# rafaelhuntstokes/bayesian_optimisation

Measured on AMD Instinct MI355X. Metric: candidate acquisitions/sec, higher is better.
Workload: dtype f64

## Files before the change

bayesian_optimisation_amd/_lib.py:

```python
from __future__ import annotations

import ctypes as C
import os

_HERE = os.path.dirname(os.path.abspath(__file__))
LIB_PATH = os.environ.get("GPBO_LIB") or os.path.join(_HERE, "libgpbo.so")

GPBO_OK = 0
ACQ_LCB = 0
ACQ_EI = 1
NPAD = 128
CHUNK_GRANULE = 512
MAX_D = 16
MAX_D_ANY = 1024
I8_MAX_N = 16384
BATCH_MAX_Q = 64
FANTASY_BELIEVER = 0
FANTASY_LIE = 1
REFINE_MAX_P = 4096
TS_MAX_PATHS = 64
TS_MAX_FEATURES = 16384
HYPER_MEAN = 1
HYPER_SCALE = 2
HYPER_CELLS_MAX_N = 64
# ... 48 lines not shown
    "gpbo_qei_workspace_bytes": (_i64, [_i64, _i64, _i64]),
    "gpbo_posterior_qei_f64": (C.c_int, [_p, _i64, _p, _i64, _i64, _i32, _p, _p, _p, _f64, _f64, _f64, _p, _i32, _i64,
                                         _i64, _p, _p, _p, _i64, _p, _p]),
    "gpbo_padded_n_f32": (_i64, [_i64]),
    "gpbo_prepare_f32": (C.c_int, [_p, _p, _i64, _p, _p, _i64, _p]),
    "gpbo_posterior_workspace_bytes_f32": (_i64, [_i64, _i64, _i64]),
    "gpbo_posterior_acq_f32": (C.c_int, [_p, _i64, _p, _i64, _i64, _i32, _p, _p, _p, _f64, _i32, _f64, _f64, _f64,
                                         _i64, _i64, _p, _p, _p, _p, _p, _p, _i64, _p, _p]),
    "gpbo_prepare_i8_bytes": (_i64, [_i64]),
    "gpbo_prepare_i8": (C.c_int, [_p, _i64, _p, _i64, _p]),
    "gpbo_posterior_workspace_bytes_i8": (_i64, [_i64, _i64, _i64]),
    "gpbo_posterior_acq_i8": (C.c_int, [_p, _i64, _p, _i64, _i64, _i32, _p, _p, _p, _f64, _i32, _f64, _f64, _i64, _i64,
                                        _p, _p, _p, _p, _p, _p, _i64, _p, _p]),
    "gpbo_posterior_acq_i8c": (C.c_int, [_p, _i64, _p, _i64, _i64, _i32, _p, _p, _p, _f64, _i32, _f64, _f64, _i64, _i64,
                                         _p, _p, _p, _p, _p, _p, _i64, _p, _p]),
    "gpbo_posterior_prefix_f64": (C.c_int, [_p, _i64, _p, _i64, _i64, _i32, _p, _p, _p, _f64, _i32, _f64, _f64, _i64, _i64,
                                            _i64, _p, _p, _p, _p, _p, _i64, _p, _p]),
    "gpbo_bound_select_f64": (C.c_int, [_p, _i64, _p, _p, _i64, _i64, _i32, _p, _p, _p, _f64, _i32, _f64, _f64, _i64,
                                        _i64, _i64, _i64, _i64, _p, _p, _p, _i64, _p]),
    "gpbo_fps_order_workspace_bytes": (_i64, [_i64]),
    "gpbo_fps_order_f64": (C.c_int, [_p, _p, _i64, _i32, _p, _i64, _p, _p, _p, _p, _i64, _p]),
    "gpbo_fps_order_status": (C.c_int, [_p, _i64, _p, _p]),
    "gpbo_rescore_workspace_bytes": (_i64, [_i64, _i64, _i64]),
    "gpbo_rescore_f64": (C.c_int, [_p, _i64, _p, _p, _p, _i64, _i64, _i32, _p, _p, _p, _f64, _i32, _f64, _f64, _i64,
                                   _f64, _i64, _i64, _i64, _p, _p, _p, _i64, _p]),
    "gpbo_batch_workspace_bytes": (_i64, [_i64, _i64, _i32]),
    "gpbo_select_batch_f64": (C.c_int, [_p, _i64, _p, _i64, _i64, _i32, _p, _p, _p, _f64, _f64, _f64, _i32, _f64, _f64, _i32,
                                        _i32, _f64, _p, _p, _i64, _p, _p, _p, _p, _p, _i64, _p]),
    "gpbo_select_batch_host_f64": (C.c_int, [_p, _p, _i64, _i32, _p, _f64, _f64, _p, _i64, _i32, _f64, _f64, _i64, _i32, _i32,
                                             _f64, _p, _p, _p, _p, _p, _p]),
    "gpbo_posterior_grad_workspace_bytes": (_i64, [_i64, _i64]),
    "gpbo_posterior_grad_f64": (C.c_int, [_p, _i64, _p, _i64, _i64, _i32, _p, _p, _p, _f64, _i32, _f64, _f64, _p, _p, _p, _p, _p,
                                          _p, _p, _i64, _p]),
    "gpbo_refine_workspace_bytes": (_i64, [_i64, _i64]),
    "gpbo_refine_f64": (C.c_int, [_p, _i64, _p, _p, _p, _i64, _i64, _i32, _p, _p, _p, _f64, _i32, _f64, _f64, _i32, _f64, _p, _p,
                                  _p, _p, _p, _p, _i64, _p]),
    "gpbo_refine_host_f64": (C.c_int, [_p, _p, _i64, _i32, _p, _f64, _f64, _p, _i64, _p, _p, _i32, _f64, _f64, _i32, _f64, _p, _p,
                                       _p, _p, _p, _p]),
    "gpbo_thompson_weights_workspace_bytes": (_i64, [_i64, _i32, _i32]),
    "gpbo_thompson_weights_f64": (C.c_int, [_p, _p, _i64, _i64, _i32, _p, _p, _f64, _f64, _p, _p, _p, _p, _i32, _i32, _p, _p, _i64,
                                            _p]),
    "gpbo_thompson_paths_workspace_bytes": (_i64, [_i64, _i64, _i32, _i32]),
    "gpbo_thompson_paths_f64": (C.c_int, [_p, _i64, _p, _i64, _i64, _i32, _p, _p, _p, _p, _p, _i32, _i32, _i64, _p, _i64, _p, _p,
                                          _p, _p, _i64, _p]),
    "gpbo_thompson_host_f64": (C.c_int, [_p, _p, _i64, _i32, _p, _f64, _f64, _p, _i64, _p, _p, _p, _p, _i32, _i32, _p, _p, _p, _p,
                                         _p]),
# ... 119 lines not shown
```

bayesian_optimisation_amd/csrc/rescore.hip:

```cpp
#include "gpbo_internal.h"

#include <limits>

namespace {

constexpr int SB = 256;

__device__ __forceinline__ void bounds(int kind, double mu, double var, double tau, double p0, double p1, double &lo,
                                       double &hi) {
    const double a = fabs(var);
    const double s_lo = sqrt(fmax(a - tau, 0.0)), s_hi = sqrt(a + tau);
    const double a_lo = gpbo_acquisition(kind, mu, s_lo, p0, p1);
    const double a_hi = gpbo_acquisition(kind, mu, s_hi, p0, p1);
    lo = (a_hi < a_lo) ? a_hi : a_lo;
    hi = (a_hi < a_lo) ? a_lo : a_hi;
}

__global__ __launch_bounds__(SB) void screen_lo_kernel(const double *__restrict__ mu, const double *__restrict__ var,
                                                       int64_t M, double tau, int kind, double p0, double p1,
                                                       double *__restrict__ part) {
    __shared__ double s_val[SB / 64];
    double best = -std::numeric_limits<double>::infinity();
    for (int64_t c = (int64_t)blockIdx.x * SB + threadIdx.x; c < M; c += (int64_t)gridDim.x * SB) {
        double lo, hi;
// ... 35 lines not shown
    const int lane = threadIdx.x & 63;
    const int64_t step = (int64_t)gridDim.x * SB;
    const int64_t cmax = (M + step - 1) / step * step;
    for (int64_t c = (int64_t)blockIdx.x * SB + threadIdx.x; c < cmax; c += step) {
        bool keep = false;
        if (c < M) {
            double lo, hi;
            bounds(kind, mu[c], var[c], tau, p0, p1, lo, hi);
            keep = !(hi < thr) || (c % stride) == 0;
        }
        const unsigned long long m = __ballot(keep);
        if (m) {
            unsigned long long base = 0;
            if (lane == 0) base = atomicAdd(count, (unsigned long long)__popcll(m));
            base = __shfl(base, 0);
            if (keep) {
                const unsigned long long pos = base + __popcll(m & ((1ull << lane) - 1ull));
                if ((int64_t)pos < cap) list[pos] = c;
            }
        }
    }
}

__global__ __launch_bounds__(SB) void bound_select_kernel(const double *__restrict__ ub, int64_t M, double thr, double slack,
                                                          int64_t stride, int64_t *__restrict__ list, int64_t cap,
                                                          unsigned long long *__restrict__ count) {
    __shared__ unsigned s_cnt[SB];
    __shared__ unsigned long long s_base;
    const int64_t step = (int64_t)gridDim.x * SB;
    unsigned mine = 0;
    for (int64_t c = (int64_t)blockIdx.x * SB + threadIdx.x; c < M; c += step)
        mine += (!(ub[c] + slack < thr) || (c % stride) == 0) ? 1u : 0u;
    s_cnt[threadIdx.x] = mine;
    __syncthreads();
    if (threadIdx.x == 0) {
        unsigned tot = 0;
        for (int t = 0; t < SB; ++t) { const unsigned v = s_cnt[t]; s_cnt[t] = tot; tot += v; }
        s_base = tot ? atomicAdd(count, (unsigned long long)tot) : 0ull;
    }
    __syncthreads();
    if (!list || !mine) return;
    unsigned long long pos = s_base + s_cnt[threadIdx.x];
    for (int64_t c = (int64_t)blockIdx.x * SB + threadIdx.x; c < M; c += step)
        if (!(ub[c] + slack < thr) || (c % stride) == 0) {
            if ((int64_t)pos < cap) list[pos] = c;
            ++pos;
        }
}

__global__ __launch_bounds__(SB) void bound_minmax_kernel(const double *__restrict__ ub, int64_t M, double *__restrict__ part) {
    __shared__ double s_hi[SB / 64], s_lo[SB / 64];
    double hi = -std::numeric_limits<double>::infinity(), lo = std::numeric_limits<double>::infinity();
    for (int64_t c = (int64_t)blockIdx.x * SB + threadIdx.x; c < M; c += (int64_t)gridDim.x * SB) {
        const double v = ub[c];
        if (v > hi) hi = v;
        if (v < lo) lo = v;
    }
#pragma unroll
    for (int off = 1; off < 64; off <<= 1) {
        hi = fmax(hi, __shfl_xor(hi, off));
        lo = fmin(lo, __shfl_xor(lo, off));
    }
    if ((threadIdx.x & 63) == 0) { s_hi[threadIdx.x >> 6] = hi; s_lo[threadIdx.x >> 6] = lo; }
    __syncthreads();
    if (threadIdx.x == 0) {
        for (int w = 1; w < SB / 64; ++w) { hi = fmax(hi, s_hi[w]); lo = fmin(lo, s_lo[w]); }
        part[blockIdx.x] = hi;
        part[gridDim.x + blockIdx.x] = lo;
    }
}

__global__ __launch_bounds__(SB) void bound_minmax_finish_kernel(const double *__restrict__ part, int n, double *__restrict__ out2) {
    __shared__ double s_hi[SB / 64], s_lo[SB / 64];
    double hi = -std::numeric_limits<double>::infinity(), lo = std::numeric_limits<double>::infinity();
    for (int i = threadIdx.x; i < n; i += SB) { hi = fmax(hi, part[i]); lo = fmin(lo, part[n + i]); }
#pragma unroll
    for (int off = 1; off < 64; off <<= 1) {
        hi = fmax(hi, __shfl_xor(hi, off));
        lo = fmin(lo, __shfl_xor(lo, off));
    }
    if ((threadIdx.x & 63) == 0) { s_hi[threadIdx.x >> 6] = hi; s_lo[threadIdx.x >> 6] = lo; }
    __syncthreads();
    if (threadIdx.x == 0) {
        for (int w = 1; w < SB / 64; ++w) { hi = fmax(hi, s_hi[w]); lo = fmin(lo, s_lo[w]); }
        out2[0] = hi;
        out2[1] = lo;
    }
}

__global__ __launch_bounds__(SB) void bound_refine_kernel(const double *__restrict__ ub2, const int64_t *__restrict__ list,
                                                          int64_t K, double thr, double slack, int64_t *__restrict__ list_out,
                                                          unsigned long long *__restrict__ count) {
    const int lane = threadIdx.x & 63;
    const int64_t step = (int64_t)gridDim.x * SB;
    const int64_t imax = (K + step - 1) / step * step;
    for (int64_t i = (int64_t)blockIdx.x * SB + threadIdx.x; i < imax; i += step) {
        const bool keep = i < K && !(ub2[i] + slack < thr);
        const unsigned long long m = __ballot(keep);
        if (m) {
            unsigned long long base = 0;
            if (lane == 0) base = atomicAdd(count, (unsigned long long)__popcll(m));
            base = __shfl(base, 0);
            if (keep) list_out[base + __popcll(m & ((1ull << lane) - 1ull))] = list[i];
        }
    }
}

__global__ __launch_bounds__(SB) void gather_rows_kernel(const double *__restrict__ Xs, int d, const int64_t *__restrict__ list,
                                                         int64_t K, double *__restrict__ out) {
    const int64_t e = (int64_t)blockIdx.x * SB + threadIdx.x;
    if (e >= K * d) return;
    const int64_t i = e / d;
    out[e] = Xs[list[i] * d + (e - i * d)];
}

// ... 28 lines not shown
        err = fmax(err, __shfl_xor(err, off));
        nans += __shfl_xor(nans, off);
    }
    const int w = threadIdx.x >> 6;
    if ((threadIdx.x & 63) == 0) { s_err[w] = err; s_nan[w] = nans; }
    gpbo_argmax_post(bv, bi, threadIdx.x & 63, w, s_val, s_idx);
    __syncthreads();
    if (threadIdx.x == 0) {
        gpbo_argmax_fold(s_val, s_idx, SB / 64, bv, bi);
        for (int q = 1; q < SB / 64; ++q) {
            err = fmax(err, s_err[q]);
            nans += s_nan[q];
        }
        out->res.best_val = bv;
        out->res.best_idx = bi;
        out->res.nan_count = (int64_t)nans;
        out->res.reserved = 0;
        out->err_max = err;
        out->pad = 0.0;
    }
}

struct RescoreLayout {
    int64_t part_off, L_off, count_off, list_off, rows_off, mu_off, sig_off, acq_off, out_off, post_off, post_bytes, total;
};

constexpr int SCREEN_BLOCKS = 1024;

RescoreLayout rescore_layout(int64_t Np, int64_t cap, int64_t chunk64) {
    RescoreLayout L;
    int64_t off = 0;
    L.part_off = off; off += align_up((int64_t)sizeof(double) * SCREEN_BLOCKS, 256);
    L.L_off = off; off += 256;
    L.count_off = off; off += 256;
    L.out_off = off; off += 256;
    L.list_off = off; off += align_up((int64_t)sizeof(int64_t) * cap, 256);
    L.rows_off = off; off += align_up((int64_t)sizeof(double) * cap * GPBO_MAX_D, 256);
    L.mu_off = off; off += align_up((int64_t)sizeof(double) * cap, 256);
    L.sig_off = off; off += align_up((int64_t)sizeof(double) * cap, 256);
    L.acq_off = off; off += align_up((int64_t)sizeof(double) * cap, 256);
    L.post_off = off;
    L.post_bytes = gpbo_posterior_workspace_bytes_split(Np, chunk64, cap, GPBO_RESCORE_SPLIT_MAX);
    off += align_up(L.post_bytes, 256);
    L.total = off;
    return L;
}

struct RescoreWork {
    double *part, *Ldev;
    unsigned long long *count;
    RescoreOut *out;
    int64_t *list;
    double *rows, *mu64, *sig64, *acq64;
    void *post;
    int64_t post_bytes;
    RescoreWork(void *work, const RescoreLayout &L) {
        char *w = reinterpret_cast<char *>(work);
        part = reinterpret_cast<double *>(w + L.part_off);
        Ldev = reinterpret_cast<double *>(w + L.L_off);
        count = reinterpret_cast<unsigned long long *>(w + L.count_off);
        out = reinterpret_cast<RescoreOut *>(w + L.out_off);
        list = reinterpret_cast<int64_t *>(w + L.list_off);
        rows = reinterpret_cast<double *>(w + L.rows_off);
        mu64 = reinterpret_cast<double *>(w + L.mu_off);
        sig64 = reinterpret_cast<double *>(w + L.sig_off);
        acq64 = reinterpret_cast<double *>(w + L.acq_off);
        post = w + L.post_off;
        post_bytes = L.post_bytes;
    }
};

bool read_back(void *dst_host, const void *src, size_t bytes, hipStream_t st) {
    return hipMemcpyAsync(dst_host, src, bytes, hipMemcpyDeviceToHost, st) == hipSuccess &&
           hipStreamSynchronize(st) == hipSuccess;
}

int score_list(const double *Xs, const GpModel &gp, const Acquisition &acq, int64_t chunk64, const RescoreWork &W, int64_t K,
               int64_t n_prefix, const DenseOut &dense, void *stream) {
    const int64_t tot = K * gp.d;
    hipLaunchKernelGGL(gather_rows_kernel, dim3((unsigned)((tot + SB - 1) / SB)), dim3(SB), 0, gpbo_stream(stream), Xs,
                       (int)gp.d, W.list, K, W.rows);
    GPBO_CHECK_LAUNCH();
    return gpbo_posterior_acq_f64_split(W.rows, K, gp, acq, 0.0, 0, clamp_chunk(chunk64, K), dense, &W.out->res, W.post,
                                        W.post_bytes, nullptr, GPBO_RESCORE_SPLIT_MAX, n_prefix, stream);
}

}

extern "C" int64_t gpbo_rescore_workspace_bytes(int64_t Np, int64_t cap, int64_t chunk64) {
    if (cap < 1 || gpbo_posterior_workspace_bytes(Np, chunk64, cap) < 0) return GPBO_ERR_ARG;
// ... 59 lines not shown
    stt.fallback = 1;
    *stats_host = stt;
    return GPBO_OK;
}

extern "C" int gpbo_bound_select_f64(const double *Xs, int64_t M, const double *ub, const double *X, int64_t N, int64_t Np,
                                     int32_t d, const double *ls_host, const double *U, const double *alpha,
                                     double prior_var, int32_t acq_kind, double p0, double p1, int64_t idx_offset,
                                     int64_t sample_stride, int64_t cap, int64_t chunk64, int64_t n_prefix2,
                                     gpbo_result *result, gpbo_screen_stats *stats_host, void *work, int64_t work_bytes,
                                     void *stream) {
    if (!Xs || !ub || !X || !U || !alpha || !result || !stats_host || !work) return GPBO_ERR_ARG;
    if (n_prefix2 < 0 || n_prefix2 > Np || n_prefix2 % 128) return GPBO_ERR_ARG;
    if (M < 1 || N < 1 || Np != gpbo_padded_n(N) || d < 1 || d > GPBO_MAX_D || cap < 1 || sample_stride < 1) return GPBO_ERR_ARG;
    if (!acq_kind_ok(acq_kind)) return GPBO_ERR_ARG;
    if (acq_kind == GPBO_ACQ_LCB && !(p0 >= 0.0)) return GPBO_ERR_ARG;
    if (gpbo_posterior_workspace_bytes(Np, chunk64, cap) < 0 || !aligned_to(work, 256)) return GPBO_ERR_ARG;
    const RescoreLayout L = rescore_layout(Np, cap, chunk64);
    if (work_bytes < L.total) return GPBO_ERR_WORKSPACE;
    hipStream_t st = gpbo_stream(stream);
    const GpModel gp = {X, N, Np, d, ls_host, U, alpha, prior_var};
    const Acquisition acq = {acq_kind, p0, p1};
    const RescoreWork W(work, L);
    double *const part = W.part, *const Ldev = W.Ldev, *const mu64 = W.mu64, *const sig64 = W.sig64, *const acq64 = W.acq64;
    unsigned long long *const count = W.count;
    RescoreOut *const out = W.out;
    int64_t *const list = W.list;
    int64_t nblk = (M + SB - 1) / SB;
    if (nblk > SCREEN_BLOCKS) nblk = SCREEN_BLOCKS;
    const double inf = std::numeric_limits<double>::infinity();
    gpbo_screen_stats stt = {0, 0, 0, 0, 0.0, 0.0};

    auto exact = [&](int64_t K, RescoreOut *h) -> int {
        int rc = score_list(Xs, gp, acq, chunk64, W, K, 0, {mu64, sig64, acq64, nullptr}, stream);
        if (rc != GPBO_OK) return rc;
        hipLaunchKernelGGL(rescore_finish_kernel, dim3(1), dim3(SB), 0, st, acq64, sig64, list, K, (const double *)nullptr,
                           idx_offset, out);
        GPBO_CHECK_LAUNCH();
        if (!read_back(h, out, sizeof(*h), st)) return GPBO_ERR_LAUNCH;
        stt.rescored += K;
        ++stt.rounds;
        return GPBO_OK;
    };
    const int64_t no_sample = std::numeric_limits<int64_t>::max();
    auto select = [&](double thr, int64_t stride, unsigned long long *K, bool count_only = false) -> int {
        if (hipMemsetAsync(count, 0, sizeof(unsigned long long), st) != hipSuccess) return GPBO_ERR_LAUNCH;
        const double slack = (thr == inf) ? 0.0 : 1e-10 * fmax(1.0, fabs(thr));
        hipLaunchKernelGGL(bound_select_kernel, dim3((unsigned)nblk), dim3(SB), 0, st, ub, M, thr, slack, stride,
                           count_only ? (int64_t *)nullptr : list, cap, count);
        GPBO_CHECK_LAUNCH();
        return read_back(K, count, sizeof(*K), st) ? GPBO_OK : GPBO_ERR_LAUNCH;
    };

    RescoreOut h;
    unsigned long long K = 0;
    int rc;
    double thr = -inf;
    auto minmax = [&](const double *v, int64_t n, double *mm) -> int {
        int64_t blk = (n + SB - 1) / SB;
        if (blk > SCREEN_BLOCKS / 2) blk = SCREEN_BLOCKS / 2;
        hipLaunchKernelGGL(bound_minmax_kernel, dim3((unsigned)blk), dim3(SB), 0, st, v, n, part);
        hipLaunchKernelGGL(bound_minmax_finish_kernel, dim3(1), dim3(SB), 0, st, part, (int)blk, Ldev);
        GPBO_CHECK_LAUNCH();
        return read_back(mm, Ldev, 2 * sizeof(double), st) ? GPBO_OK : GPBO_ERR_LAUNCH;
    };
    auto bisect = [&](const double *mm, int64_t want_lo, int64_t want_hi, auto &&counter, double *level) -> int {
        *level = inf;
        if (!(mm[0] > mm[1]) || !(mm[0] < inf) || !(mm[1] > -inf)) return GPBO_OK;
        double lo = mm[1], hi = mm[0];
        for (int it = 0; it < 30; ++it) {
            const double mid = 0.5 * (lo + hi);
            if (!(mid > lo) || !(mid < hi)) break;
            unsigned long long c = 0;
            int r = counter(mid, &c);
            if (r != GPBO_OK) return r;
            if ((int64_t)c > want_hi) lo = mid;
            else if ((int64_t)c < want_lo) hi = mid;
            else { *level = mid; break; }
        }
        return GPBO_OK;
    };
    auto count_ub = [&](double level, unsigned long long *c) -> int { return select(level, no_sample, c, true); };
    const int64_t want_hi = cap < 4096 ? cap : 4096, want_lo = want_hi / 8;
    double mm[2] = {0.0, 0.0};
    rc = minmax(ub, M, mm);
    if (rc != GPBO_OK) return rc;

    if (n_prefix2 > 0) {
        int64_t k1 = M / 64;
        if (k1 < 2048) k1 = 2048;
        if (k1 > cap / 2) k1 = cap / 2;
        double level1 = inf;
        rc = bisect(mm, k1 - k1 / 3, k1 + k1 / 2, count_ub, &level1);
        if (rc != GPBO_OK) return rc;
        if (level1 < inf) {
            rc = select(level1, no_sample, &K);
            if (rc != GPBO_OK) return rc;
            const int64_t K1 = (int64_t)K;
            if (K1 >= 1 && K1 <= cap) {
                double *ub2 = sig64;
                rc = score_list(Xs, gp, acq, chunk64, W, K1, n_prefix2, {nullptr, nullptr, ub2, nullptr}, stream);
                if (rc != GPBO_OK) return rc;
                int64_t *list2 = reinterpret_cast<int64_t *>(mu64);
                int64_t rblk = (K1 + SB - 1) / SB;
                if (rblk > SCREEN_BLOCKS) rblk = SCREEN_BLOCKS;
                auto refine_ub2 = [&](double level, unsigned long long *c) -> int {
                    if (hipMemsetAsync(count, 0, sizeof(unsigned long long), st) != hipSuccess) return GPBO_ERR_LAUNCH;
                    hipLaunchKernelGGL(bound_refine_kernel, dim3((unsigned)rblk), dim3(SB), 0, st, ub2, list, K1, level,
                                       1e-10 * fmax(1.0, fabs(level)), list2, count);
                    GPBO_CHECK_LAUNCH();
                    return read_back(c, count, sizeof(*c), st) ? GPBO_OK : GPBO_ERR_LAUNCH;
                };
                double mm2[2], level2 = inf;
                rc = minmax(ub2, K1, mm2);
                if (rc != GPBO_OK) return rc;
                const int64_t t_hi = K1 < 1024 ? K1 : 1024;
                rc = bisect(mm2, t_hi / 4, t_hi, refine_ub2, &level2);
                if (rc != GPBO_OK) return rc;
                if (level2 < inf) {
                    unsigned long long KT = 0;
                    rc = refine_ub2(level2, &KT);
                    if (rc != GPBO_OK) return rc;
                    if (KT >= 1 && (int64_t)KT <= cap) {
                        if (hipMemcpyAsync(list, list2, sizeof(int64_t) * KT, hipMemcpyDeviceToDevice, st) != hipSuccess)
                            return GPBO_ERR_LAUNCH;
                        rc = exact((int64_t)KT, &h);
                        if (rc != GPBO_OK) return rc;
                        thr = h.res.best_val;
                        stt.survivors = K1;
                        stt.tau = thr;
                        if (thr >= level1 && thr >= level2) {
                            if (hipMemcpyAsync(result, &out->res, sizeof(gpbo_result), hipMemcpyDeviceToDevice, st) != hipSuccess)
                                return GPBO_ERR_LAUNCH;
                            *stats_host = stt;
                            return GPBO_OK;
                        }
                    }
                }
            }
        }
    }

    if (!(thr > -inf)) {
        double level = inf;
        rc = bisect(mm, want_lo, want_hi, count_ub, &level);
        if (rc != GPBO_OK) return rc;
        if (level < inf) {
            rc = select(level, no_sample, &K);
            if (rc != GPBO_OK) return rc;
            if ((int64_t)K >= 1 && (int64_t)K <= cap) {
                rc = exact((int64_t)K, &h);
                if (rc != GPBO_OK) return rc;
                thr = h.res.best_val;
            }
        }
    }
    if (!(thr > -inf)) {
        rc = select(inf, sample_stride, &K);
        if (rc != GPBO_OK) return rc;
        stt.survivors = (int64_t)K;
        if ((int64_t)K > cap) { stt.fallback = 1; *stats_host = stt; return GPBO_OK; }
        rc = exact((int64_t)K, &h);
        if (rc != GPBO_OK) return rc;
        thr = h.res.best_val;
    }
    const int64_t refine = cap < 4096 ? cap : 4096;
    for (int round = 1; round <= 4; ++round) {
        stt.tau = thr;
        rc = select(thr, no_sample, &K);
        if (rc != GPBO_OK) return rc;
        stt.survivors = (int64_t)K;
        if ((int64_t)K <= cap) {
            if (n_prefix2 > 0 && (int64_t)K > 4 * refine) {
                rc = score_list(Xs, gp, acq, chunk64, W, (int64_t)K, n_prefix2, {nullptr, nullptr, acq64, nullptr}, stream);
                if (rc != GPBO_OK) return rc;
                int64_t *list2 = reinterpret_cast<int64_t *>(mu64);
                if (hipMemsetAsync(count, 0, sizeof(unsigned long long), st) != hipSuccess) return GPBO_ERR_LAUNCH;
                int64_t rblk = ((int64_t)K + SB - 1) / SB;
                if (rblk > SCREEN_BLOCKS) rblk = SCREEN_BLOCKS;
                hipLaunchKernelGGL(bound_refine_kernel, dim3((unsigned)rblk), dim3(SB), 0, st, acq64, list, (int64_t)K, thr,
                                   1e-10 * fmax(1.0, fabs(thr)), list2, count);
                GPBO_CHECK_LAUNCH();
                unsigned long long K2 = 0;
                if (!read_back(&K2, count, sizeof(K2), st)) return GPBO_ERR_LAUNCH;
                if (K2 > K) return GPBO_ERR_LAUNCH;
                if (hipMemcpyAsync(list, list2, sizeof(int64_t) * K2, hipMemcpyDeviceToDevice, st) != hipSuccess)
                    return GPBO_ERR_LAUNCH;
                K = K2;
                if (K == 0) return GPBO_ERR_LAUNCH;
            }
            if ((int64_t)K > M / 8 && (int64_t)K > 4 * refine) break;
            rc = exact((int64_t)K, &h);
            if (rc != GPBO_OK) return rc;
            if (hipMemcpyAsync(result, &out->res, sizeof(gpbo_result), hipMemcpyDeviceToDevice, st) != hipSuccess)
                return GPBO_ERR_LAUNCH;
            *stats_host = stt;
            return GPBO_OK;
        }
        if (round == 4) break;
        rc = exact(refine, &h);
        if (rc != GPBO_OK) return rc;
        if (!(h.res.best_val > thr)) break;
        thr = h.res.best_val;
    }
    stt.fallback = 1;
    *stats_host = stt;
    return GPBO_OK;
}
```

bayesian_optimisation_amd/gp_device.py:

```python
from __future__ import annotations

import ctypes as C
from contextlib import contextmanager
from dataclasses import dataclass
from typing import Optional

import numpy as np

from . import _lib, ard_fit
from .model import JITTER_ASSEMBLY, JITTER_KERNEL, need_se

NAN_ACQUISITION = "index 0 is out of bounds for axis 0 with size 0 (acquisition contains NaN)"
PRIOR_VAR = (1.0 + JITTER_KERNEL) + JITTER_ASSEMBLY

DEFAULT_CHUNK = 1 << 17


def _torch():
    if _lib.hip_used_before_pytorch:
        raise _lib.GpboError(
            "libgpbo.so was used in this process before PyTorch was imported (PointSelectorHost / host_binding first). "
            "A process that needs both must `import torch` before its first use of bayesian_optimisation_amd.")
    import torch

# ... 448 lines not shown

        need_se(self.kernel, "save_state()")
        path = str(path)
        if not path.endswith(".npz"):
            path += ".npz"
        fd, tmp = tempfile.mkstemp(prefix=".gpbo_state_", suffix=".tmp", dir=os.path.dirname(os.path.abspath(path)))
        try:
            with os.fdopen(fd, "wb") as f:
                np.savez(f, **self.state_dict())
            um = os.umask(0)
            os.umask(um)
            os.chmod(tmp, 0o666 & ~um)
            os.replace(tmp, path)
        except BaseException:
            if os.path.exists(tmp):
                os.unlink(tmp)
            raise

    def load_state(self, path: str):
        need_se(self.kernel, "load_state()")
        with np.load(path) as z:
            return self.load_state_dict({k: z[k] for k in z.files})

    def _ensure_post_workspace(self, M):
        chunk = self._chunk_for(M)
        need = int(self.lib.gpbo_posterior_workspace_bytes(self.Np, chunk, M))
        self._workspace("_work_post", need)
        return chunk, need

    def score_async(self, Xs, acquisition: str = "lcb", explore: float = 4.0, f_best: Optional[float] = None,
                    xi: float = 0.0, dense: bool = False, idx_offset: int = 0, diag_add: float = 0.0,
                    prior_var: float = PRIOR_VAR):
        torch = self.torch
        Xsd, M = self._candidates(Xs)
        kind, p0, p1 = acq_params(acquisition, explore, f_best, xi)
        if diag_add != 0.0 and self.perm is not None:
            raise ValueError("diag_add (the N == M shape quirk) needs factorise(order='arrival')")
        if diag_add != 0.0 and self.kernel != "se":
            raise ValueError(f"diag_add (the N == M shape quirk of the reference's kernel_rbf) is not available with "
                             f"kernel={self.kernel!r}")
        with torch.cuda.device(self.device):
            chunk, wbytes = self._ensure_post_workspace(M)
            mu = sigma = acq = None
            if dense:
                mu = torch.empty(M, dtype=torch.float64, device=self.device)
                sigma = torch.empty(M, dtype=torch.float64, device=self.device)
                acq = torch.empty(M, dtype=torch.float64, device=self.device)
            st = self.lib.gpbo_posterior_acq_kern_f64(
# ... 116 lines not shown

    def score_async_i8(self, Xs, acquisition: str = "lcb", explore: float = 4.0, f_best: Optional[float] = None,
                       xi: float = 0.0, dense: bool = False, idx_offset: int = 0, diag_add: float = 0.0,
                       prior_var: float = PRIOR_VAR):
        return self._score_screened("i8", Xs, acquisition, explore, f_best, xi, dense, idx_offset, diag_add, prior_var)

    def score_i8(self, Xs, **kw) -> ScoreResult:
        return self._read(self.score_async_i8(Xs, **kw))

    def score_async_i8c(self, Xs, acquisition: str = "lcb", explore: float = 4.0, f_best: Optional[float] = None,
                        xi: float = 0.0, dense: bool = False, idx_offset: int = 0, diag_add: float = 0.0,
                        prior_var: float = PRIOR_VAR):
        return self._score_screened("i8c", Xs, acquisition, explore, f_best, xi, dense, idx_offset, diag_add, prior_var)

    def score_i8c(self, Xs, **kw) -> ScoreResult:
        return self._read(self.score_async_i8c(Xs, **kw))

    def score_f32(self, Xs, **kw) -> ScoreResult:
        return self._read(self.score_async_f32(Xs, **kw))

    ARD_KEEP_WORKSPACE_BYTES = 1 << 28
    def score_async_bound(self, Xs, acquisition: str = "lcb", explore: float = 4.0, f_best: Optional[float] = None,
                          xi: float = 0.0, dense: bool = False, idx_offset: int = 0, diag_add: float = 0.0,
                          prior_var: float = PRIOR_VAR, prefix: Optional[int] = None, prefix2: Optional[int] = None):
        need_se(self.kernel, "score_bound()")
        torch = self.torch
        if self.d > _lib.MAX_D:
            self.last_screen = dict(mode="bound", fallback=True, reason="d > 16")
            return self.score_async(Xs, acquisition, explore, f_best, xi, dense, idx_offset, diag_add, prior_var)
        Xsd, M = self._candidates(Xs)
        kind, p0, p1 = acq_params(acquisition, explore, f_best, xi)
        J = int(prefix) if prefix else self.bound_prefix()
        J2 = int(prefix2) if prefix2 is not None else (4 * J if 8 * J <= self.Np else 0)
        reason = None
        if dense:
            reason = "dense outputs"
        elif diag_add != 0.0:
            reason = "diag_add"
        elif kind == _lib.ACQ_LCB and not p0 >= 0.0:
            reason = "negative explore weight"
        elif J % 128 or J < 128 or 2 * J > self.Np:
            reason = "too few column blocks"
        elif not (self.jitter1 + self.jitter2 >= self.BOUND_MIN_JITTER
                  and prior_var >= (1.0 + self.jitter1) + self.jitter2 - 1e-15):
            reason = "jitter too small for the |var| rule"
        if reason:
            self.last_screen = dict(mode="bound", fallback=True, reason=reason)
            return self.score_async(Xsd, acquisition, explore, f_best, xi, dense, idx_offset, diag_add, prior_var)
        with torch.cuda.device(self.device):
            chunk, wbytes = self._ensure_post_workspace(M)
            if self._bound_ub is None or self._bound_ub.numel() < M:
                self._bound_ub = torch.empty(M, dtype=torch.float64, device=self.device)
            lsp = self.ls_h.ctypes.data_as(C.c_void_p)
            st = self.lib.gpbo_posterior_prefix_f64(
                self._ptr(Xsd), M, self._ptr(self.X), self.N, self.Np, self.d, lsp, self._ptr(self.U),
                self._ptr(self.alpha), prior_var, kind, p0, p1, int(idx_offset), chunk, J, None, None,
                self._ptr(self._bound_ub), self._ptr(self._result), self._ptr(self._work_post), wbytes,
                self._profile if self.profile_active else None, self._stream())
            _lib.check(st, "gpbo_posterior_prefix_f64")
            cap = self.screen_cap if self.screen_cap else max(4096, M)
            chunk64 = self.SCREEN_CHUNK64
            rbytes = int(self.lib.gpbo_rescore_workspace_bytes(self.Np, cap, chunk64))
            self._workspace("_work_rescore", rbytes)
            stats = _lib.ScreenStats()
            stride = max(1, M // self.SCREEN_SAMPLE)
            st = self.lib.gpbo_bound_select_f64(
                self._ptr(Xsd), M, self._ptr(self._bound_ub), self._ptr(self.X), self.N, self.Np, self.d, lsp,
                self._ptr(self.U), self._ptr(self.alpha), prior_var, kind, p0, p1, int(idx_offset), stride, cap,
                chunk64, J2, self._ptr(self._result), C.byref(stats), self._ptr(self._work_rescore), rbytes,
                self._stream())
            _lib.check(st, "gpbo_bound_select_f64")
            self.last_screen = dict(mode="bound", order="arrival (fps fell back)" if self.order_fell_back() else self.order, prefix=J, prefix2=J2, survivors=int(stats.survivors),
                                    rescored=int(stats.rescored), rounds=int(stats.rounds), fallback=bool(stats.fallback),
# ... 526 lines not shown
```

include/gpbo.h:

```cpp
#ifndef GPBO_H
#define GPBO_H

#include <stdint.h>

#ifdef __cplusplus
extern "C" {
#endif

#define GPBO_VERSION 151


#define GPBO_OK 0
#define GPBO_ERR_ARG (-1)
#define GPBO_ERR_LAUNCH (-2)
#define GPBO_ERR_WORKSPACE (-3)

#define GPBO_MAX_D 16
#define GPBO_MAX_D_ANY 1024
#define GPBO_NPAD 128
#define GPBO_CHUNK_GRANULE 512
#define GPBO_CHUNK_MAX (1 << 24)

#define GPBO_KERNEL_SE 0
#define GPBO_KERNEL_MATERN32 1
// ... 91 lines not shown
    int64_t rescored;
    int32_t rounds;
    int32_t fallback;
    double tau;
    double err_max;
} gpbo_screen_stats;
int64_t gpbo_rescore_workspace_bytes(int64_t Np, int64_t cap, int64_t chunk64);
int gpbo_rescore_f64(const double *Xs, int64_t M, const double *mu, const double *var32, const double *X, int64_t N,
                     int64_t Np, int32_t d, const double *ls_host, const double *U, const double *alpha,
                     double prior_var, int32_t acq_kind, double p0, double p1, int64_t idx_offset, double tau0,
                     int64_t sample_stride, int64_t cap, int64_t chunk64, gpbo_result *result,
                     gpbo_screen_stats *stats_host, void *work, int64_t work_bytes, void *stream);

int gpbo_posterior_prefix_f64(const double *Xs, int64_t M, const double *X, int64_t N, int64_t Np, int32_t d,
                              const double *ls_host, const double *U, const double *alpha, double prior_var,
                              int32_t acq_kind, double p0, double p1, int64_t idx_offset, int64_t chunk, int64_t n_prefix,
                              double *mu_out, double *sigma_ub_out, double *acq_ub_out, gpbo_result *result, void *work,
                              int64_t work_bytes, gpbo_profile *prof , void *stream);
int gpbo_bound_select_f64(const double *Xs, int64_t M, const double *acq_ub, const double *X, int64_t N, int64_t Np,
                          int32_t d, const double *ls_host, const double *U, const double *alpha, double prior_var,
                          int32_t acq_kind, double p0, double p1, int64_t idx_offset, int64_t sample_stride, int64_t cap,
                          int64_t chunk64, int64_t n_prefix2 , gpbo_result *result,
                          gpbo_screen_stats *stats_host, void *work, int64_t work_bytes, void *stream);

int64_t gpbo_fps_order_workspace_bytes(int64_t N);
int gpbo_fps_order_f64(const double *X, const double *y, int64_t N, int32_t d, const double *ls_host, int64_t J,
                       int64_t *perm_out, double *Xp_out, double *yp_out, void *work, int64_t work_bytes, void *stream);
int gpbo_fps_order_status(const void *work, int64_t N, int32_t *fell_back, void *stream);

#define GPBO_I8_MAX_N 16384
int64_t gpbo_prepare_i8_bytes(int64_t Np);
int gpbo_prepare_i8(const double *U, int64_t Np, void *u8, int64_t u8_bytes, void *stream);
int64_t gpbo_posterior_workspace_bytes_i8(int64_t Np, int64_t chunk, int64_t M);
int gpbo_posterior_acq_i8(const double *Xs, int64_t M, const double *X, int64_t N, int64_t Np, int32_t d,
                          const double *ls_host, const void *u8, const double *alpha, double prior_var,
                          int32_t acq_kind, double p0, double p1, int64_t idx_offset, int64_t chunk, double *mu_out,
                          double *sigma_out, double *acq_out, double *var_out, gpbo_result *result, void *work,
                          int64_t work_bytes, gpbo_profile *prof , void *stream);
int gpbo_posterior_acq_i8c(const double *Xs, int64_t M, const double *X, int64_t N, int64_t Np, int32_t d,
                           const double *ls_host, const void *u8, const double *alpha, double prior_var,
                           int32_t acq_kind, double p0, double p1, int64_t idx_offset, int64_t chunk, double *mu_out,
                           double *sigma_out, double *acq_out, double *var_out, gpbo_result *result, void *work,
                           int64_t work_bytes, gpbo_profile *prof , void *stream);

int64_t gpbo_acq_workspace_bytes(void);
int gpbo_acq_argmax_f64(const double *mu, const double *sigma, int64_t M, int32_t acq_kind, double p0, double p1,
// ... 163 lines not shown
```

Before: 4.297 million.

## Move threshold bisection on-device with multi-level probe tree

Replaces the host-driven bisection, which did a kernel launch and host readback per probe, with a device-resident level search. Each probe kernel evaluates a 31-node bisection tree at once, so 30 probes take 6 launches, and the final selection kernel reads the level straight from device state, leaving one readback per select. This removes many host-device synchronisations in the bound-select and refine path. The trade is that each probe pass does 31 comparisons per element and always runs all rounds even after the level is found.

After: 4.294 million. About the same (-0.1%).

```diff
diff --git a/bayesian_optimisation_amd/_lib.py b/bayesian_optimisation_amd/_lib.py
--- a/bayesian_optimisation_amd/_lib.py
+++ b/bayesian_optimisation_amd/_lib.py
@@ -94,6 +94,7 @@
     "gpbo_fps_order_f64": (C.c_int, [_p, _p, _i64, _i32, _p, _i64, _p, _p, _p, _p, _i64, _p]),
     "gpbo_fps_order_status": (C.c_int, [_p, _i64, _p, _p]),
     "gpbo_rescore_workspace_bytes": (_i64, [_i64, _i64, _i64]),
+    "gpbo_bound_level_f64": (C.c_int, [_p, _i64, _i64, _i64, _p, _p, _i64, _p]),
     "gpbo_rescore_f64": (C.c_int, [_p, _i64, _p, _p, _p, _i64, _i64, _i32, _p, _p, _p, _f64, _i32, _f64, _f64, _i64,
                                    _f64, _i64, _i64, _i64, _p, _p, _p, _i64, _p]),
     "gpbo_batch_workspace_bytes": (_i64, [_i64, _i64, _i32]),
diff --git a/bayesian_optimisation_amd/csrc/rescore.hip b/bayesian_optimisation_amd/csrc/rescore.hip
--- a/bayesian_optimisation_amd/csrc/rescore.hip
+++ b/bayesian_optimisation_amd/csrc/rescore.hip
@@ -81,31 +81,18 @@
     }
 }
 
-__global__ __launch_bounds__(SB) void bound_select_kernel(const double *__restrict__ ub, int64_t M, double thr, double slack,
-                                                          int64_t stride, int64_t *__restrict__ list, int64_t cap,
-                                                          unsigned long long *__restrict__ count) {
-    __shared__ unsigned s_cnt[SB];
-    __shared__ unsigned long long s_base;
-    const int64_t step = (int64_t)gridDim.x * SB;
-    unsigned mine = 0;
-    for (int64_t c = (int64_t)blockIdx.x * SB + threadIdx.x; c < M; c += step)
-        mine += (!(ub[c] + slack < thr) || (c % stride) == 0) ? 1u : 0u;
-    s_cnt[threadIdx.x] = mine;
-    __syncthreads();
-    if (threadIdx.x == 0) {
-        unsigned tot = 0;
-        for (int t = 0; t < SB; ++t) { const unsigned v = s_cnt[t]; s_cnt[t] = tot; tot += v; }
-        s_base = tot ? atomicAdd(count, (unsigned long long)tot) : 0ull;
-    }
-    __syncthreads();
-    if (!list || !mine) return;
-    unsigned long long pos = s_base + s_cnt[threadIdx.x];
-    for (int64_t c = (int64_t)blockIdx.x * SB + threadIdx.x; c < M; c += step)
-        if (!(ub[c] + slack < thr) || (c % stride) == 0) {
-            if ((int64_t)pos < cap) list[pos] = c;
-            ++pos;
-        }
-}
+struct LevelState {
+    double level;
+    unsigned long long count;
+    unsigned long long listed;
+    double lo, hi;
+    int probes, done, found;
+};
+constexpr int TREE_DEPTH = 5, TREE_NODES = (1 << TREE_DEPTH) - 1, LEVEL_PROBES = 30, LEVEL_BLOCKS = 512;
+constexpr int64_t LEVEL_COUNT_OFF = 256, LEVEL_PART_OFF = 512;
+constexpr int64_t LEVEL_BYTES = LEVEL_PART_OFF + (int64_t)sizeof(double) * 2 * LEVEL_BLOCKS;
+static_assert(sizeof(LevelState) <= 256 && LEVEL_BYTES == GPBO_BOUND_LEVEL_WORKSPACE_BYTES, "level workspace");
+static_assert(LEVEL_PROBES % TREE_DEPTH == 0 && (TREE_NODES + 1) * sizeof(unsigned long long) <= 256, "level workspace");
 
 __global__ __launch_bounds__(SB) void bound_minmax_kernel(const double *__restrict__ ub, int64_t M, double *__restrict__ part) {
     __shared__ double s_hi[SB / 64], s_lo[SB / 64];
@@ -129,7 +116,7 @@
     }
 }
 
-__global__ __launch_bounds__(SB) void bound_minmax_finish_kernel(const double *__restrict__ part, int n, double *__restrict__ out2) {
+__global__ __launch_bounds__(SB) void level_begin_kernel(const double *__restrict__ part, int n, LevelState *__restrict__ state) {
     __shared__ double s_hi[SB / 64], s_lo[SB / 64];
     double hi = -std::numeric_limits<double>::infinity(), lo = std::numeric_limits<double>::infinity();
     for (int i = threadIdx.x; i < n; i += SB) { hi = fmax(hi, part[i]); lo = fmin(lo, part[n + i]); }
@@ -142,14 +129,142 @@
     __syncthreads();
     if (threadIdx.x == 0) {
         for (int w = 1; w < SB / 64; ++w) { hi = fmax(hi, s_hi[w]); lo = fmin(lo, s_lo[w]); }
-        out2[0] = hi;
-        out2[1] = lo;
-    }
+        const double inf = std::numeric_limits<double>::infinity();
+        state->lo = lo;
+        state->hi = hi;
+        state->level = inf;
+        if (!(hi > lo) || !(hi < inf) || !(lo > -inf)) state->done = 1;
+    }
+}
+
+__global__ __launch_bounds__(SB) void level_probe_kernel(const double *__restrict__ v, int64_t n, int64_t want_lo, int64_t want_hi,
+                                                         LevelState *__restrict__ state, unsigned long long *__restrict__ counts) {
+    __shared__ double s_lo[TREE_NODES], s_hi[TREE_NODES], s_mid[TREE_NODES], s_slack[TREE_NODES];
+    __shared__ unsigned s_cnt[TREE_NODES];
+    __shared__ bool s_last;
+    if (state->done) return;
+    if (threadIdx.x == 0) {
+        s_lo[0] = state->lo;
+        s_hi[0] = state->hi;
+        for (int i = 0; i < TREE_NODES; ++i) {
+            const double mid = 0.5 * (s_lo[i] + s_hi[i]);
+            s_mid[i] = mid;
+            s_slack[i] = 1e-10 * fmax(1.0, fabs(mid));
+            if (2 * i + 2 < TREE_NODES) {
+                s_lo[2 * i + 1] = mid; s_hi[2 * i + 1] = s_hi[i];
+                s_lo[2 * i + 2] = s_lo[i]; s_hi[2 * i + 2] = mid;
+            }
+        }
+    }
+    if (threadIdx.x < TREE_NODES) s_cnt[threadIdx.x] = 0u;
+    __syncthreads();
+    unsigned cnt[TREE_NODES];
+#pragma unroll
+    for (int j = 0; j < TREE_NODES; ++j) cnt[j] = 0u;
+    for (int64_t c = (int64_t)blockIdx.x * SB + threadIdx.x; c < n; c += (int64_t)gridDim.x * SB) {
+        const double x = v[c];
+#pragma unroll
+        for (int j = 0; j < TREE_NODES; ++j) cnt[j] += !(x + s_slack[j] < s_mid[j]) ? 1u : 0u;
+    }
+#pragma unroll
+    for (int j = 0; j < TREE_NODES; ++j) {
+        unsigned t = cnt[j];
+#pragma unroll
+        for (int off = 1; off < 64; off <<= 1) t += __shfl_xor(t, off);
+        if ((threadIdx.x & 63) == 0 && t) atomicAdd(&s_cnt[j], t);
+    }
+    __syncthreads();
+    if (threadIdx.x < TREE_NODES && s_cnt[threadIdx.x]) atomicAdd(&counts[threadIdx.x], (unsigned long long)s_cnt[threadIdx.x]);
+    __threadfence();
+    __syncthreads();
+    if (threadIdx.x == 0) s_last = atomicAdd(&counts[TREE_NODES], 1ull) == (unsigned long long)gridDim.x - 1ull;
+    __syncthreads();
+    if (!s_last) return;
+    __threadfence();
+    __shared__ unsigned long long s_tot[TREE_NODES];
+    if (threadIdx.x < TREE_NODES) s_tot[threadIdx.x] = atomicExch(&counts[threadIdx.x], 0ull);
+    if (threadIdx.x == TREE_NODES) atomicExch(&counts[TREE_NODES], 0ull);
+    __syncthreads();
+    if (threadIdx.x != 0) return;
+    int node = 0, probes = state->probes;
+    for (int depth = 0; depth < TREE_DEPTH; ++depth, ++probes) {
+        const double lo = s_lo[node], hi = s_hi[node], mid = s_mid[node];
+        if (probes >= LEVEL_PROBES || !(mid > lo) || !(mid < hi)) { state->done = 1; return; }
+        const unsigned long long c = s_tot[node];
+        if ((int64_t)c > want_hi) node = 2 * node + 1;
+        else if ((int64_t)c < want_lo) node = 2 * node + 2;
+        else {
+            state->level = mid;
+            state->count = c;
+            state->found = 1;
+            state->done = 1;
+            return;
+        }
+        if (depth + 1 == TREE_DEPTH) {
+            state->lo = (int64_t)c > want_hi ? mid : lo;
+            state->hi = (int64_t)c > want_hi ? hi : mid;
+        }
+    }
+    state->probes = probes;
+    if (probes >= LEVEL_PROBES) state->done = 1;
+}
+
+int find_level(const double *v, int64_t n, int64_t want_lo, int64_t want_hi, void *level_work, hipStream_t st) {
+    char *w = reinterpret_cast<char *>(level_work);
+    LevelState *state = reinterpret_cast<LevelState *>(w);
+    unsigned long long *counts = reinterpret_cast<unsigned long long *>(w + LEVEL_COUNT_OFF);
+    double *part = reinterpret_cast<double *>(w + LEVEL_PART_OFF);
+    if (hipMemsetAsync(level_work, 0, LEVEL_PART_OFF, st) != hipSuccess) return GPBO_ERR_LAUNCH;
+    int64_t blk = (n + SB - 1) / SB;
+    if (blk > LEVEL_BLOCKS) blk = LEVEL_BLOCKS;
+    hipLaunchKernelGGL(bound_minmax_kernel, dim3((unsigned)blk), dim3(SB), 0, st, v, n, part);
+    hipLaunchKernelGGL(level_begin_kernel, dim3(1), dim3(SB), 0, st, part, (int)blk, state);
+    for (int r = 0; r < LEVEL_PROBES / TREE_DEPTH; ++r)
+        hipLaunchKernelGGL(level_probe_kernel, dim3((unsigned)blk), dim3(SB), 0, st, v, n, want_lo, want_hi, state, counts);
+    GPBO_CHECK_LAUNCH();
+    return GPBO_OK;
+}
+
+__global__ __launch_bounds__(SB) void bound_select_kernel(const double *__restrict__ ub, int64_t M, double thr,
+                                                          const LevelState *__restrict__ lv, int64_t stride,
+                                                          int64_t *__restrict__ list, int64_t cap,
+                                                          unsigned long long *__restrict__ count) {
+    __shared__ unsigned s_cnt[SB];
+    __shared__ unsigned long long s_base;
+    if (lv) {
+        if (!lv->found) return;
+        thr = lv->level;
+    }
+    const double slack = (thr == std::numeric_limits<double>::infinity()) ? 0.0 : 1e-10 * fmax(1.0, fabs(thr));
+    const int64_t step = (int64_t)gridDim.x * SB;
+    unsigned mine = 0;
+    for (int64_t c = (int64_t)blockIdx.x * SB + threadIdx.x; c < M; c += step)
+        mine += (!(ub[c] + slack < thr) || (c % stride) == 0) ? 1u : 0u;
+    s_cnt[threadIdx.x] = mine;
+    __syncthreads();
+    if (threadIdx.x == 0) {
+        unsigned tot = 0;
+        for (int t = 0; t < SB; ++t) { const unsigned v = s_cnt[t]; s_cnt[t] = tot; tot += v; }
+        s_base = tot ? atomicAdd(count, (unsigned long long)tot) : 0ull;
+    }
+    __syncthreads();
+    if (!mine) return;
+    unsigned long long pos = s_base + s_cnt[threadIdx.x];
+    for (int64_t c = (int64_t)blockIdx.x * SB + threadIdx.x; c < M; c += step)
+        if (!(ub[c] + slack < thr) || (c % stride) == 0) {
+            if ((int64_t)pos < cap) list[pos] = c;
+            ++pos;
+        }
 }
 
 __global__ __launch_bounds__(SB) void bound_refine_kernel(const double *__restrict__ ub2, const int64_t *__restrict__ list,
-                                                          int64_t K, double thr, double slack, int64_t *__restrict__ list_out,
-                                                          unsigned long long *__restrict__ count) {
+                                                          int64_t K, double thr, const LevelState *__restrict__ lv,
+                                                          int64_t *__restrict__ list_out, unsigned long long *__restrict__ count) {
+    if (lv) {
+        if (!lv->found) return;
+        thr = lv->level;
+    }
+    const double slack = 1e-10 * fmax(1.0, fabs(thr));
     const int lane = threadIdx.x & 63;
     const int64_t step = (int64_t)gridDim.x * SB;
     const int64_t imax = (K + step - 1) / step * step;
@@ -224,7 +339,7 @@
 }
 
 struct RescoreLayout {
-    int64_t part_off, L_off, count_off, list_off, rows_off, mu_off, sig_off, acq_off, out_off, post_off, post_bytes, total;
+    int64_t part_off, L_off, count_off, level_off, list_off, rows_off, mu_off, sig_off, acq_off, out_off, post_off, post_bytes, total;
 };
 
 constexpr int SCREEN_BLOCKS = 1024;
@@ -236,6 +351,7 @@
     L.L_off = off; off += 256;
     L.count_off = off; off += 256;
     L.out_off = off; off += 256;
+    L.level_off = off; off += align_up(LEVEL_BYTES, 256);
     L.list_off = off; off += align_up((int64_t)sizeof(int64_t) * cap, 256);
     L.rows_off = off; off += align_up((int64_t)sizeof(double) * cap * GPBO_MAX_D, 256);
     L.mu_off = off; off += align_up((int64_t)sizeof(double) * cap, 256);
@@ -254,7 +370,7 @@
     RescoreOut *out;
     int64_t *list;
     double *rows, *mu64, *sig64, *acq64;
-    void *post;
+    void *post, *level;
     int64_t post_bytes;
     RescoreWork(void *work, const RescoreLayout &L) {
         char *w = reinterpret_cast<char *>(work);
@@ -268,6 +384,7 @@
         sig64 = reinterpret_cast<double *>(w + L.sig_off);
         acq64 = reinterpret_cast<double *>(w + L.acq_off);
         post = w + L.post_off;
+        level = w + L.level_off;
         post_bytes = L.post_bytes;
     }
 };
@@ -373,7 +490,7 @@
     const GpModel gp = {X, N, Np, d, ls_host, U, alpha, prior_var};
     const Acquisition acq = {acq_kind, p0, p1};
     const RescoreWork W(work, L);
-    double *const part = W.part, *const Ldev = W.Ldev, *const mu64 = W.mu64, *const sig64 = W.sig64, *const acq64 = W.acq64;
+    double *const mu64 = W.mu64, *const sig64 = W.sig64, *const acq64 = W.acq64;
     unsigned long long *const count = W.count;
     RescoreOut *const out = W.out;
     int64_t *const list = W.list;
@@ -394,116 +511,79 @@
         return GPBO_OK;
     };
     const int64_t no_sample = std::numeric_limits<int64_t>::max();
-    auto select = [&](double thr, int64_t stride, unsigned long long *K, bool count_only = false) -> int {
+    auto select = [&](double thr, int64_t stride, unsigned long long *K) -> int {
         if (hipMemsetAsync(count, 0, sizeof(unsigned long long), st) != hipSuccess) return GPBO_ERR_LAUNCH;
-        const double slack = (thr == inf) ? 0.0 : 1e-10 * fmax(1.0, fabs(thr));
-        hipLaunchKernelGGL(bound_select_kernel, dim3((unsigned)nblk), dim3(SB), 0, st, ub, M, thr, slack, stride,
-                           count_only ? (int64_t *)nullptr : list, cap, count);
+        hipLaunchKernelGGL(bound_select_kernel, dim3((unsigned)nblk), dim3(SB), 0, st, ub, M, thr, (const LevelState *)nullptr,
+                           stride, list, cap, count);
         GPBO_CHECK_LAUNCH();
         return read_back(K, count, sizeof(*K), st) ? GPBO_OK : GPBO_ERR_LAUNCH;
     };
+    LevelState *const lvdev = reinterpret_cast<LevelState *>(W.level);
+    auto select_level = [&](int64_t want_lo, int64_t want_hi, LevelState *lv) -> int {
+        int r = find_level(ub, M, want_lo, want_hi, W.level, st);
+        if (r != GPBO_OK) return r;
+        hipLaunchKernelGGL(bound_select_kernel, dim3((unsigned)nblk), dim3(SB), 0, st, ub, M, 0.0, (const LevelState *)lvdev,
+                           no_sample, list, cap, &lvdev->listed);
+        GPBO_CHECK_LAUNCH();
+        return read_back(lv, lvdev, sizeof(*lv), st) ? GPBO_OK : GPBO_ERR_LAUNCH;
+    };
 
     RescoreOut h;
+    LevelState lv;
     unsigned long long K = 0;
     int rc;
     double thr = -inf;
-    auto minmax = [&](const double *v, int64_t n, double *mm) -> int {
-        int64_t blk = (n + SB - 1) / SB;
-        if (blk > SCREEN_BLOCKS / 2) blk = SCREEN_BLOCKS / 2;
-        hipLaunchKernelGGL(bound_minmax_kernel, dim3((unsigned)blk), dim3(SB), 0, st, v, n, part);
-        hipLaunchKernelGGL(bound_minmax_finish_kernel, dim3(1), dim3(SB), 0, st, part, (int)blk, Ldev);
-        GPBO_CHECK_LAUNCH();
-        return read_back(mm, Ldev, 2 * sizeof(double), st) ? GPBO_OK : GPBO_ERR_LAUNCH;
-    };
-    auto bisect = [&](const double *mm, int64_t want_lo, int64_t want_hi, auto &&counter, double *level) -> int {
-        *level = inf;
-        if (!(mm[0] > mm[1]) || !(mm[0] < inf) || !(mm[1] > -inf)) return GPBO_OK;
-        double lo = mm[1], hi = mm[0];
-        for (int it = 0; it < 30; ++it) {
-            const double mid = 0.5 * (lo + hi);
-            if (!(mid > lo) || !(mid < hi)) break;
-            unsigned long long c = 0;
-            int r = counter(mid, &c);
-            if (r != GPBO_OK) return r;
-            if ((int64_t)c > want_hi) lo = mid;
-            else if ((int64_t)c < want_lo) hi = mid;
-            else { *level = mid; break; }
-        }
-        return GPBO_OK;
-    };
-    auto count_ub = [&](double level, unsigned long long *c) -> int { return select(level, no_sample, c, true); };
     const int64_t want_hi = cap < 4096 ? cap : 4096, want_lo = want_hi / 8;
-    double mm[2] = {0.0, 0.0};
-    rc = minmax(ub, M, mm);
-    if (rc != GPBO_OK) return rc;
 
     if (n_prefix2 > 0) {
         int64_t k1 = M / 64;
         if (k1 < 2048) k1 = 2048;
         if (k1 > cap / 2) k1 = cap / 2;
-        double level1 = inf;
-        rc = bisect(mm, k1 - k1 / 3, k1 + k1 / 2, count_ub, &level1);
-        if (rc != GPBO_OK) return rc;
-        if (level1 < inf) {
-            rc = select(level1, no_sample, &K);
+        rc = select_level(k1 - k1 / 3, k1 + k1 / 2, &lv);
+        if (rc != GPBO_OK) return rc;
+        const double level1 = lv.level;
+        const int64_t K1 = (int64_t)lv.listed;
+        if (lv.found && K1 >= 1 && K1 <= cap) {
+            double *ub2 = sig64;
+            rc = score_list(Xs, gp, acq, chunk64, W, K1, n_prefix2, {nullptr, nullptr, ub2, nullptr}, stream);
             if (rc != GPBO_OK) return rc;
-            const int64_t K1 = (int64_t)K;
-            if (K1 >= 1 && K1 <= cap) {
-                double *ub2 = sig64;
-                rc = score_list(Xs, gp, acq, chunk64, W, K1, n_prefix2, {nullptr, nullptr, ub2, nullptr}, stream);
+            int64_t *list2 = reinterpret_cast<int64_t *>(mu64);
+            int64_t rblk = (K1 + SB - 1) / SB;
+            if (rblk > SCREEN_BLOCKS) rblk = SCREEN_BLOCKS;
+            const int64_t t_hi = K1 < 1024 ? K1 : 1024;
+            rc = find_level(ub2, K1, t_hi / 4, t_hi, W.level, st);
+            if (rc != GPBO_OK) return rc;
+            hipLaunchKernelGGL(bound_refine_kernel, dim3((unsigned)rblk), dim3(SB), 0, st, ub2, list, K1, 0.0,
+                               (const LevelState *)lvdev, list2, &lvdev->listed);
+            GPBO_CHECK_LAUNCH();
+            if (!read_back(&lv, lvdev, sizeof(lv), st)) return GPBO_ERR_LAUNCH;
+            const double level2 = lv.level;
+            const int64_t KT = (int64_t)lv.listed;
+            if (lv.found && KT >= 1 && KT <= cap) {
+                if (hipMemcpyAsync(list, list2, sizeof(int64_t) * KT, hipMemcpyDeviceToDevice, st) != hipSuccess)
+                    return GPBO_ERR_LAUNCH;
+                rc = exact(KT, &h);
                 if (rc != GPBO_OK) return rc;
-                int64_t *list2 = reinterpret_cast<int64_t *>(mu64);
-                int64_t rblk = (K1 + SB - 1) / SB;
-                if (rblk > SCREEN_BLOCKS) rblk = SCREEN_BLOCKS;
-                auto refine_ub2 = [&](double level, unsigned long long *c) -> int {
-                    if (hipMemsetAsync(count, 0, sizeof(unsigned long long), st) != hipSuccess) return GPBO_ERR_LAUNCH;
-                    hipLaunchKernelGGL(bound_refine_kernel, dim3((unsigned)rblk), dim3(SB), 0, st, ub2, list, K1, level,
-                                       1e-10 * fmax(1.0, fabs(level)), list2, count);
-                    GPBO_CHECK_LAUNCH();
-                    return read_back(c, count, sizeof(*c), st) ? GPBO_OK : GPBO_ERR_LAUNCH;
-                };
-                double mm2[2], level2 = inf;
-                rc = minmax(ub2, K1, mm2);
-                if (rc != GPBO_OK) return rc;
-                const int64_t t_hi = K1 < 1024 ? K1 : 1024;
-                rc = bisect(mm2, t_hi / 4, t_hi, refine_ub2, &level2);
-                if (rc != GPBO_OK) return rc;
-                if (level2 < inf) {
-                    unsigned long long KT = 0;
-                    rc = refine_ub2(level2, &KT);
-                    if (rc != GPBO_OK) return rc;
-                    if (KT >= 1 && (int64_t)KT <= cap) {
-                        if (hipMemcpyAsync(list, list2, sizeof(int64_t) * KT, hipMemcpyDeviceToDevice, st) != hipSuccess)
-                            return GPBO_ERR_LAUNCH;
-                        rc = exact((int64_t)KT, &h);
-                        if (rc != GPBO_OK) return rc;
-                        thr = h.res.best_val;
-                        stt.survivors = K1;
-                        stt.tau = thr;
-                        if (thr >= level1 && thr >= level2) {
-                            if (hipMemcpyAsync(result, &out->res, sizeof(gpbo_result), hipMemcpyDeviceToDevice, st) != hipSuccess)
-                                return GPBO_ERR_LAUNCH;
-                            *stats_host = stt;
-                            return GPBO_OK;
-                        }
-                    }
+                thr = h.res.best_val;
+                stt.survivors = K1;
+                stt.tau = thr;
+                if (thr >= level1 && thr >= level2) {
+                    if (hipMemcpyAsync(result, &out->res, sizeof(gpbo_result), hipMemcpyDeviceToDevice, st) != hipSuccess)
+                        return GPBO_ERR_LAUNCH;
+                    *stats_host = stt;
+                    return GPBO_OK;
                 }
             }
         }
     }
 
     if (!(thr > -inf)) {
-        double level = inf;
-        rc = bisect(mm, want_lo, want_hi, count_ub, &level);
-        if (rc != GPBO_OK) return rc;
-        if (level < inf) {
-            rc = select(level, no_sample, &K);
+        rc = select_level(want_lo, want_hi, &lv);
+        if (rc != GPBO_OK) return rc;
+        if (lv.found && (int64_t)lv.listed >= 1 && (int64_t)lv.listed <= cap) {
+            rc = exact((int64_t)lv.listed, &h);
             if (rc != GPBO_OK) return rc;
-            if ((int64_t)K >= 1 && (int64_t)K <= cap) {
-                rc = exact((int64_t)K, &h);
-                if (rc != GPBO_OK) return rc;
-                thr = h.res.best_val;
-            }
+            thr = h.res.best_val;
         }
     }
     if (!(thr > -inf)) {
@@ -530,7 +610,7 @@
                 int64_t rblk = ((int64_t)K + SB - 1) / SB;
                 if (rblk > SCREEN_BLOCKS) rblk = SCREEN_BLOCKS;
                 hipLaunchKernelGGL(bound_refine_kernel, dim3((unsigned)rblk), dim3(SB), 0, st, acq64, list, (int64_t)K, thr,
-                                   1e-10 * fmax(1.0, fabs(thr)), list2, count);
+                                   (const LevelState *)nullptr, list2, count);
                 GPBO_CHECK_LAUNCH();
                 unsigned long long K2 = 0;
                 if (!read_back(&K2, count, sizeof(K2), st)) return GPBO_ERR_LAUNCH;
@@ -558,3 +638,14 @@
     *stats_host = stt;
     return GPBO_OK;
 }
+
+extern "C" int gpbo_bound_level_f64(const double *ub, int64_t n, int64_t want_lo, int64_t want_hi, void *out, void *work,
+                                    int64_t work_bytes, void *stream) {
+    if (!ub || !out || !work || n < 1 || want_lo < 0 || want_hi < want_lo) return GPBO_ERR_ARG;
+    if (!aligned_to(work, 256) || !aligned_to(out, 8)) return GPBO_ERR_ARG;
+    if (work_bytes < LEVEL_BYTES) return GPBO_ERR_WORKSPACE;
+    hipStream_t st = gpbo_stream(stream);
+    int rc = find_level(ub, n, want_lo, want_hi, work, st);
+    if (rc != GPBO_OK) return rc;
+    return hipMemcpyAsync(out, work, 16, hipMemcpyDeviceToDevice, st) == hipSuccess ? GPBO_OK : GPBO_ERR_LAUNCH;
+}
diff --git a/bayesian_optimisation_amd/gp_device.py b/bayesian_optimisation_amd/gp_device.py
--- a/bayesian_optimisation_amd/gp_device.py
+++ b/bayesian_optimisation_amd/gp_device.py
@@ -494,8 +494,10 @@
         with np.load(path) as z:
             return self.load_state_dict({k: z[k] for k in z.files})
 
-    def _ensure_post_workspace(self, M):
-        chunk = self._chunk_for(M)
+    def _ensure_post_workspace(self, M, chunk=None):
+        if chunk is not None and (chunk < _lib.CHUNK_GRANULE or chunk % _lib.CHUNK_GRANULE):
+            raise ValueError(f"chunk must be a positive multiple of {_lib.CHUNK_GRANULE}")
+        chunk = self._chunk_for(M) if chunk is None else min(int(chunk), _round_up(M, _lib.CHUNK_GRANULE))
         need = int(self.lib.gpbo_posterior_workspace_bytes(self.Np, chunk, M))
         self._workspace("_work_post", need)
         return chunk, need
@@ -658,7 +660,8 @@
     ARD_KEEP_WORKSPACE_BYTES = 1 << 28
     def score_async_bound(self, Xs, acquisition: str = "lcb", explore: float = 4.0, f_best: Optional[float] = None,
                           xi: float = 0.0, dense: bool = False, idx_offset: int = 0, diag_add: float = 0.0,
-                          prior_var: float = PRIOR_VAR, prefix: Optional[int] = None, prefix2: Optional[int] = None):
+                          prior_var: float = PRIOR_VAR, prefix: Optional[int] = None, prefix2: Optional[int] = None,
+                          chunk: Optional[int] = None):
         need_se(self.kernel, "score_bound()")
         torch = self.torch
         if self.d > _lib.MAX_D:
@@ -684,7 +687,7 @@
             self.last_screen = dict(mode="bound", fallback=True, reason=reason)
             return self.score_async(Xsd, acquisition, explore, f_best, xi, dense, idx_offset, diag_add, prior_var)
         with torch.cuda.device(self.device):
-            chunk, wbytes = self._ensure_post_workspace(M)
+            chunk, wbytes = self._ensure_post_workspace(M, chunk)
             if self._bound_ub is None or self._bound_ub.numel() < M:
                 self._bound_ub = torch.empty(M, dtype=torch.float64, device=self.device)
             lsp = self.ls_h.ctypes.data_as(C.c_void_p)
diff --git a/include/gpbo.h b/include/gpbo.h
--- a/include/gpbo.h
+++ b/include/gpbo.h
@@ -137,6 +137,9 @@
                           int32_t acq_kind, double p0, double p1, int64_t idx_offset, int64_t sample_stride, int64_t cap,
                           int64_t chunk64, int64_t n_prefix2 , gpbo_result *result,
                           gpbo_screen_stats *stats_host, void *work, int64_t work_bytes, void *stream);
+#define GPBO_BOUND_LEVEL_WORKSPACE_BYTES 8704
+int gpbo_bound_level_f64(const double *ub, int64_t n, int64_t want_lo, int64_t want_hi, void *out, void *work,
+                         int64_t work_bytes, void *stream);
 
 int64_t gpbo_fps_order_workspace_bytes(int64_t N);
 int gpbo_fps_order_f64(const double *X, const double *y, int64_t N, int32_t d, const double *ls_host, int64_t J,
```
